# RobotLocomotion/pytorch-dense-correspondence

Measured on NVIDIA H100. Metric: image-pairs/s (640x480, D=3) fwd+loss+bwd, higher is better.
Workload: dtype f32 (bf16x3 split on the wgmma tensor cores, fp32 accumulate)

## Files before the change

### pytorch-dense-correspondence_b200/csrc/bn.cu

```cuda
#include "conv.cuh"

namespace ddn {

constexpr int BN_THREADS = 256;

__device__ __forceinline__ void store_split4(__nv_bfloat16* hi, __nv_bfloat16* lo, int64_t i4, float4 v) {
  __nv_bfloat16 h0 = __float2bfloat16_rn(v.x), h1 = __float2bfloat16_rn(v.y), h2 = __float2bfloat16_rn(v.z), h3 = __float2bfloat16_rn(v.w);
  __nv_bfloat162 a = __halves2bfloat162(h0, h1), b = __halves2bfloat162(h2, h3);
  uint2 ho; ho.x = *reinterpret_cast<uint32_t*>(&a); ho.y = *reinterpret_cast<uint32_t*>(&b);
  reinterpret_cast<uint2*>(hi)[i4] = ho;
  if (lo) {
    __nv_bfloat162 c = __halves2bfloat162(__float2bfloat16_rn(v.x - __bfloat162float(h0)), __float2bfloat16_rn(v.y - __bfloat162float(h1)));
    __nv_bfloat162 d = __halves2bfloat162(__float2bfloat16_rn(v.z - __bfloat162float(h2)), __float2bfloat16_rn(v.w - __bfloat162float(h3)));
    uint2 l2; l2.x = *reinterpret_cast<uint32_t*>(&c); l2.y = *reinterpret_cast<uint32_t*>(&d);
    reinterpret_cast<uint2*>(lo)[i4] = l2;
  }
}
__device__ __forceinline__ float4 bf16x4_to_float4(uint2 h) {
  return make_float4(__uint_as_float(h.x << 16), __uint_as_float(h.x & 0xffff0000u), __uint_as_float(h.y << 16),
                     __uint_as_float(h.y & 0xffff0000u));
}
__device__ __forceinline__ void mask_from_bf16x4(uint2 h, float4& g) {
  if ((h.x & 0x8000u) || !(h.x & 0x7fffu)) g.x = 0.f;
  if ((h.x & 0x80000000u) || !(h.x & 0x7fff0000u)) g.y = 0.f;
// ... 252 lines not shown
    if (a.g_out) reinterpret_cast<float4*>(a.g_out)[i] = g;
    float4 d;
    d.x = k1.x * (g.x - mb.x - (v.x - mu.x) * is.x * mg.x);
    d.y = k1.y * (g.y - mb.y - (v.y - mu.y) * is.y * mg.y);
    d.z = k1.z * (g.z - mb.z - (v.z - mu.z) * is.z * mg.z);
    d.w = k1.w * (g.w - mb.w - (v.w - mu.w) * is.w * mg.w);
    if (a.dx) reinterpret_cast<float4*>(a.dx)[i] = d;
    if (a.dx_hi) store_split4(a.dx_hi, a.dx_lo, i, d);
  }
}

__global__ void __launch_bounds__(256)
stem_bn_relu_pool_kernel(const float* __restrict__ x, const float* __restrict__ mean, const float* __restrict__ invstd,
                         const float* __restrict__ gamma, const float* __restrict__ beta,
                         float* __restrict__ y, uint8_t* __restrict__ argmax, __nv_bfloat16* __restrict__ y_hi,
                         __nv_bfloat16* __restrict__ y_lo, int N, int Hc, int Wc, int C, int Hp, int Wp, int imgs_per_group) {
  pdl_prologue();
  const int q = C >> 2;
  const int64_t total = (int64_t)N * Hp * Wp * q;
  for (int64_t i = (int64_t)blockIdx.x * blockDim.x + threadIdx.x; i < total; i += (int64_t)gridDim.x * blockDim.x) {
    int c = (int)(i % q) << 2; int64_t t = i / q;
    int wp = (int)(t % Wp); t /= Wp;
    int hp = (int)(t % Hp); int n = (int)(t / Hp);
    const int so = (n / imgs_per_group) * C + c;
    float4 mu = *reinterpret_cast<const float4*>(mean + so), is = *reinterpret_cast<const float4*>(invstd + so);
    float4 ga = *reinterpret_cast<const float4*>(gamma + c), be = *reinterpret_cast<const float4*>(beta + c);
    float4 sc = make_float4(ga.x * is.x, ga.y * is.y, ga.z * is.z, ga.w * is.w);
    float4 best = make_float4(-INFINITY, -INFINITY, -INFINITY, -INFINITY);
    uchar4 arg = make_uchar4(0, 0, 0, 0);
#pragma unroll
    for (int r = 0; r < 3; ++r) {
      int h = 2 * hp - 1 + r;
      if (h < 0 || h >= Hc) continue;
#pragma unroll
      for (int s = 0; s < 3; ++s) {
        int w = 2 * wp - 1 + s;
        if (w < 0 || w >= Wc) continue;
        float4 v = __ldg(reinterpret_cast<const float4*>(x + (((int64_t)n * Hc + h) * Wc + w) * C + c));
        v.x = fmaxf(fmaf(v.x - mu.x, sc.x, be.x), 0.f); v.y = fmaxf(fmaf(v.y - mu.y, sc.y, be.y), 0.f);
        v.z = fmaxf(fmaf(v.z - mu.z, sc.z, be.z), 0.f); v.w = fmaxf(fmaf(v.w - mu.w, sc.w, be.w), 0.f);
        unsigned char k = (unsigned char)(r * 3 + s);
        if (v.x > best.x) { best.x = v.x; arg.x = k; }
        if (v.y > best.y) { best.y = v.y; arg.y = k; }
        if (v.z > best.z) { best.z = v.z; arg.z = k; }
        if (v.w > best.w) { best.w = v.w; arg.w = k; }
      }
    }
    if (y) reinterpret_cast<float4*>(y)[i] = best;
    reinterpret_cast<uchar4*>(argmax)[i] = arg;
    if (y_hi) store_split4(y_hi, y_lo, i, best);
  }
}

__global__ void __launch_bounds__(256)
stem_pool_relu_bwd_kernel(const float* __restrict__ dyp, const uint8_t* __restrict__ argmax, const float* __restrict__ x,
                          const float* __restrict__ mean, const float* __restrict__ invstd,
                          const float* __restrict__ gamma, const float* __restrict__ beta, float* __restrict__ g,
                          int N, int Hc, int Wc, int C, int Hp, int Wp, int imgs_per_group) {
  pdl_prologue();
  const int q = C >> 2;
  const int64_t total = (int64_t)N * Hc * Wc * q;
  for (int64_t i = (int64_t)blockIdx.x * blockDim.x + threadIdx.x; i < total; i += (int64_t)gridDim.x * blockDim.x) {
    int c = (int)(i % q) << 2; int64_t t = i / q;
    int w = (int)(t % Wc); t /= Wc;
    int h = (int)(t % Hc); int n = (int)(t / Hc);
    float4 acc = make_float4(0, 0, 0, 0);
    int hp0 = h >> 1, hp1 = (h + 1) >> 1, wp0 = w >> 1, wp1 = (w + 1) >> 1;
#pragma unroll
    for (int a = 0; a < 2; ++a) {
      int hp = a ? hp1 : hp0;
      if ((a && hp1 == hp0) || hp >= Hp) continue;
      int r = h - (2 * hp - 1);
#pragma unroll
      for (int b = 0; b < 2; ++b) {
        int wp = b ? wp1 : wp0;
        if ((b && wp1 == wp0) || wp >= Wp) continue;
        int s = w - (2 * wp - 1);
        unsigned char k = (unsigned char)(r * 3 + s);
        int64_t pi = (((int64_t)n * Hp + hp) * Wp + wp) * q + (c >> 2);
        uchar4 am = reinterpret_cast<const uchar4*>(argmax)[pi];
        float4 d = __ldg(reinterpret_cast<const float4*>(dyp) + pi);
        if (am.x == k) acc.x += d.x;
        if (am.y == k) acc.y += d.y;
        if (am.z == k) acc.z += d.z;
        if (am.w == k) acc.w += d.w;
      }
    }
    const int so = (n / imgs_per_group) * C + c;
    float4 mu = *reinterpret_cast<const float4*>(mean + so), is = *reinterpret_cast<const float4*>(invstd + so);
    float4 ga = *reinterpret_cast<const float4*>(gamma + c), be = *reinterpret_cast<const float4*>(beta + c);
    float4 v = __ldg(reinterpret_cast<const float4*>(x) + i);
    if (!(fmaf(v.x - mu.x, ga.x * is.x, be.x) > 0.f)) acc.x = 0.f;
    if (!(fmaf(v.y - mu.y, ga.y * is.y, be.y) > 0.f)) acc.y = 0.f;
    if (!(fmaf(v.z - mu.z, ga.z * is.z, be.z) > 0.f)) acc.z = 0.f;
    if (!(fmaf(v.w - mu.w, ga.w * is.w, be.w) > 0.f)) acc.w = 0.f;
    reinterpret_cast<float4*>(g)[i] = acc;
  }
}

bool bn_c_supported(int C) {
  return C >= 4 && C % 4 == 0 && (C <= BN_COLSUM_MAX_C ? BN_THREADS % (C / 4) == 0 : (C % BN_COLSUM_MAX_C == 0 && C <= 4096));
}

static int check_c(int C, int G, int64_t M) {
  DDN_CHECK_ARG(bn_c_supported(C), "BatchNorm kernels need C in {4..1024} with 256 %% (C/4) == 0, or a multiple of 1024 up to 4096 (got %d)", C);
  DDN_CHECK_ARG(G >= 1 && G <= BN_MAX_GROUPS && M % G == 0, "BatchNorm groups: need 1 <= G <= %d dividing the row count", BN_MAX_GROUPS);
  return 0;
}
template <typename K>
static int resident_blocks(K kernel, size_t smem) {
  int per_sm = 0;
  if (cudaOccupancyMaxActiveBlocksPerMultiprocessor(&per_sm, kernel, BN_THREADS, smem) != cudaSuccess || per_sm < 1) per_sm = 4;
  return per_sm * num_sms();
}
template <typename K>
static int ew_blocks(K kernel, size_t smem, int64_t total) {
  return (int)std::min<int64_t>(ceil_div(total, BN_THREADS), (int64_t)resident_blocks(kernel, smem));
}

int launch_bn_stats(const float* x, int64_t M, int C, int G, BnAccum acc, float* mean, float* invstd,
                    float* running_mean, float* running_var, float momentum, float eps, cudaStream_t st) {
  DDN_TRY(check_c(C, G, M));
  const int64_t Mg = M / G;
  const int resident = resident_blocks(bn_colsum_kernel<0>, 0);
  const int Cs = bn_slice_c(C), slices = C / Cs;
  BnColsumArgs a = {x, nullptr, nullptr, nullptr, nullptr, nullptr, nullptr, nullptr, Mg, C, bn_colsum_rows_per_block(Mg, C, G * slices, resident), 0, Cs};
  BnFwdFinal ff = {acc, mean, invstd, running_mean, running_var, Mg, G, C, momentum, eps};
  BnBwdFinal fb = {};
  dim3 grid((unsigned)bn_colsum_blocks(Mg, C, G * slices, resident), (unsigned)G, (unsigned)slices);
  DDN_LAUNCH(bn_colsum_kernel<0>, grid, BN_THREADS, 0, st, a, ff, fb);
  return 0;
}

int launch_bn_eval_stats(const float* rm, const float* rv, int C, int G, float eps, float* mean, float* invstd, cudaStream_t st) {
  DDN_LAUNCH(bn_eval_stats_kernel, (int)ceil_div(C, 128), 128, 0, st, rm, rv, C, G, eps, mean, invstd);
  return 0;
}

int launch_bn_eval_stats_all(const float* buffers, float* stats_base, const BnEvalSeg* segs, int n_segs, int G, float eps, cudaStream_t st) {
  DDN_CHECK_ARG(n_segs >= 1, "no BatchNorm segments");
  for (int i0 = 0; i0 < n_segs; i0 += BN_EVAL_MAX_SEGS) {
    BnEvalSegs s; s.n = std::min(BN_EVAL_MAX_SEGS, n_segs - i0);
    for (int i = 0; i < s.n; ++i) s.s[i] = segs[i0 + i];
    dim3 grid(2, (unsigned)s.n);
    DDN_LAUNCH(bn_eval_stats_all_kernel, grid, 256, 0, st, buffers, stats_base, s, G, eps);
  }
  return 0;
}

int launch_bn_fold(const float* rm, const float* rv, const float* gamma, const float* beta, int C, float eps,
                   float* scale, float* shift, cudaStream_t st) {
  DDN_LAUNCH(bn_fold_kernel, (int)ceil_div(C, 128), 128, 0, st, rm, rv, gamma, beta, C, eps, scale, shift);
  return 0;
}

template <typename K>
static int allow_smem(K kernel, size_t smem) {
  if (smem > 48 * 1024) DDN_CUDA(cudaFuncSetAttribute(kernel, cudaFuncAttributeMaxDynamicSharedMemorySize, (int)smem));
  return 0;
}

int launch_bn_apply(const BnApplyArgs& a, cudaStream_t st) {
  DDN_TRY(check_c(a.C, a.G, a.M));
  const size_t smem = (size_t)a.G * ((a.r && a.rmean) ? 6 : 3) * a.C * sizeof(float);
  DDN_TRY(allow_smem(bn_apply_kernel, smem));
  DDN_LAUNCH(bn_apply_kernel, ew_blocks(bn_apply_kernel, smem, a.M * (a.C / 4)), BN_THREADS, smem, st, a);
  return 0;
}

int launch_bn_backward(const BnBwdArgs& a, cudaStream_t st) {
  DDN_TRY(check_c(a.C, a.G, a.M));
  const int64_t Mg = a.M / a.G;
  const int resident = resident_blocks(bn_colsum_kernel<1>, 0);
  const int Cs = bn_slice_c(a.C), slices = a.C / Cs;
  BnColsumArgs ca = {a.x, a.dy, a.y, a.y_hi, a.mean, a.invstd, a.gamma, a.beta, Mg, a.C, bn_colsum_rows_per_block(Mg, a.C, a.G * slices, resident),
                     a.relu, Cs};
  DDN_CHECK_ARG(!(a.relu && !a.y && !a.y_hi) || a.beta, "recomputing the ReLU mask needs beta");
  BnFwdFinal ff = {};
  BnBwdFinal fb = {a.acc, a.sums, a.dgamma, a.dbeta, a.G, a.C};
  dim3 grid((unsigned)bn_colsum_blocks(Mg, a.C, a.G * slices, resident), (unsigned)a.G, (unsigned)slices);
  if (!a.sums_ready) DDN_LAUNCH(bn_colsum_kernel<1>, grid, BN_THREADS, 0, st, ca, ff, fb);
  const size_t smem = (size_t)a.G * 7 * a.C * sizeof(float);
  DDN_TRY(allow_smem(bn_bwd_apply_kernel, smem));
  DDN_LAUNCH(bn_bwd_apply_kernel, ew_blocks(bn_bwd_apply_kernel, smem, a.M * (a.C / 4)), BN_THREADS, smem, st, a);
  return 0;
}

int launch_stem_bn_relu_pool(const float* x, const float* mean, const float* invstd, const float* gamma, const float* beta,
                             float* y, uint8_t* argmax, __nv_bfloat16* y_hi, __nv_bfloat16* y_lo,
                             int N, int Hc, int Wc, int C, int G, cudaStream_t st) {
  int Hp = (Hc - 1) / 2 + 1, Wp = (Wc - 1) / 2 + 1;
  int64_t total = (int64_t)N * Hp * Wp * (C / 4);
  DDN_LAUNCH(stem_bn_relu_pool_kernel, ew_blocks(stem_bn_relu_pool_kernel, 0, total), 256, 0, st, x, mean, invstd, gamma, beta, y, argmax, y_hi, y_lo, N, Hc, Wc, C,
             Hp, Wp, N / G);
  return 0;
}

int launch_stem_pool_relu_backward(const float* dy_pool, const uint8_t* argmax, const float* x, const float* mean,
                                   const float* invstd, const float* gamma, const float* beta, float* g,
                                   int N, int Hc, int Wc, int C, int G, cudaStream_t st) {
  int Hp = (Hc - 1) / 2 + 1, Wp = (Wc - 1) / 2 + 1;
  int64_t total = (int64_t)N * Hc * Wc * (C / 4);
  DDN_LAUNCH(stem_pool_relu_bwd_kernel, ew_blocks(stem_pool_relu_bwd_kernel, 0, total), 256, 0, st, dy_pool, argmax, x, mean, invstd, gamma, beta, g,
             N, Hc, Wc, C, Hp, Wp, N / G);
  return 0;
}

}
```

### pytorch-dense-correspondence_b200/csrc/conv.cuh

```cuda
#pragma once
#include "common.cuh"
#include "bn_stats.cuh"

namespace ddn {

struct ConvGeom {
  int N, Hin, Win, Cin;
  int Hout, Wout, Cout;
  int KH, KW;
  int stride;
  int ups;
  int pad, dil;
  int cin_log2;
};

int conv_geom_init(ConvGeom* g, int N, int Hin, int Win, int Cin, int Hout, int Wout, int Cout,
                   int KH, int KW, int stride, int ups, int pad, int dil);
int launch_pack_weights(const float* w, float* wp, int Cout, int Cin, int CinP, int KH, int KW, int dgrad, cudaStream_t st);
int launch_unpack_wgrad(const float* dwp, float* dw, int Cout, int Cin, int CinP, int KH, int KW, cudaStream_t st);
int launch_conv_gather_f32(const float* in, const float* wp, const float* addend, float* out, const ConvGeom& g, cudaStream_t st);
int launch_conv_wgrad_f32(const float* in, const float* dy, float* dwp, const ConvGeom& g, cudaStream_t st);

bool bn_c_supported(int C);
size_t bn_accum_bytes(int C);
BnAccum bn_accum_at(void* base, int C);
int launch_bn_stats(const float* x, int64_t M, int C, int G, BnAccum acc, float* mean, float* invstd,
                    float* running_mean, float* running_var, float momentum, float eps, cudaStream_t st);
struct BnEvalSeg { int64_t rm_off, rv_off, stat_off; int C; };
int launch_bn_eval_stats_all(const float* buffers, float* stats_base, const BnEvalSeg* segs, int n_segs, int G, float eps, cudaStream_t st);
int launch_bn_eval_stats(const float* running_mean, const float* running_var, int C, int G, float eps,
                         float* mean, float* invstd, cudaStream_t st);
int launch_bn_fold(const float* running_mean, const float* running_var, const float* gamma, const float* beta, int C, float eps,
                   float* scale, float* shift, cudaStream_t st);
struct BnApplyArgs {
  const float* x; const float* mean; const float* invstd; const float* gamma; const float* beta;
  const float* r; const __nv_bfloat16* r_hi; const __nv_bfloat16* r_lo;
  const float* rmean; const float* rinvstd; const float* rgamma; const float* rbeta;
  float* y; __nv_bfloat16* hi; __nv_bfloat16* lo;
  int64_t M; int C; int relu; int G;
};
int launch_bn_apply(const BnApplyArgs& a, cudaStream_t st);
struct BnBwdArgs {
  const float* dy; const float* x; const float* mean; const float* invstd; const float* gamma; const float* beta;
  const float* y; const __nv_bfloat16* y_hi;
  float* dx; __nv_bfloat16* dx_hi; __nv_bfloat16* dx_lo; float* g_out;
  float* dgamma; float* dbeta;
  BnAccum acc; float* sums;
  int64_t M; int C; int relu; int training; int G;
  int sums_ready;
};
int launch_bn_backward(const BnBwdArgs& a, cudaStream_t st);

int launch_stem_bn_relu_pool(const float* x, const float* mean, const float* invstd, const float* gamma, const float* beta,
                             float* y, uint8_t* argmax, __nv_bfloat16* y_hi, __nv_bfloat16* y_lo,
                             int N, int Hc, int Wc, int C, int G, cudaStream_t st);
int launch_stem_pool_relu_backward(const float* dy_pool, const uint8_t* argmax, const float* x, const float* mean,
                                   const float* invstd, const float* gamma, const float* beta, float* g,
                                   int N, int Hc, int Wc, int C, int G, cudaStream_t st);

int launch_nchw_to_nhwc4(const float* x, float* y, int N, int H, int W, cudaStream_t st);
int launch_fc_forward(const float* feat, const __nv_bfloat16* feat_hi, const __nv_bfloat16* feat_lo, const float* w, const float* bias,
                      float* low, float* low_nhwc, int64_t Mimg, int N, int C, int D, cudaStream_t st);
int launch_add_lowres_nhwc(const float* dlow_nhwc, float* dlow, int64_t Mimg, int N, int D, int accumulate, cudaStream_t st);
size_t fc_part_floats(int C, int D);
int launch_fc_backward(const float* dlow, const float* feat, const __nv_bfloat16* feat_hi, const __nv_bfloat16* feat_lo, const float* w,
                       float* dfeat, float* dw, float* dbias, float* part, int64_t Mimg, int N, int C, int D, cudaStream_t st);
int launch_upsample_fwd(const float* x, float* y, int NC, int h, int w, int H, int W, cudaStream_t st);
int launch_upsample_bwd(const float* dy, float* dx, int NC, int h, int w, int H, int W, cudaStream_t st);
int launch_upsample_unit_fwd(const float* x, float* y, int N, int D, int h, int w, int H, int W, cudaStream_t st);
int launch_upsample_unit_bwd(const float* x, const float* dy, float* dx, float* g, int N, int D, int h, int w, int H, int W, cudaStream_t st);
int launch_fill_zero(void* p, size_t bytes, cudaStream_t st);

}
```

### pytorch-dense-correspondence_b200/csrc/conv_tc.cu

```cuda
#include <cuda.h>
#include <algorithm>
#include <cstring>
#include <functional>
#include <mutex>
#include <unordered_map>

#include "conv.cuh"
#include "conv_tc.cuh"

namespace ddn {

constexpr int TC_BLOCK_K = 64;
constexpr int TC_CONSUMERS = 256;
constexpr int TC_THREADS = TC_CONSUMERS + 32;
constexpr int TC_PRODUCER_WARP = TC_CONSUMERS / 32;
constexpr int TC_WIDE_THREADS = TC_CONSUMERS + 128;
constexpr int TC_A_BYTES = 128 * TC_BLOCK_K * 2;

__device__ __forceinline__ uint32_t smem_u32(const void* p) { return (uint32_t)__cvta_generic_to_shared(p); }

__device__ __forceinline__ void mbar_init(uint32_t bar, uint32_t count) {
  asm volatile("mbarrier.init.shared::cta.b64 [%0], %1;" ::"r"(bar), "r"(count));
}
__device__ __forceinline__ void mbar_expect_tx(uint32_t bar, uint32_t bytes) {
// ... 169 lines not shown
  const float* addend;
  int imgs_per_group;
  BnFwdFinal fin;
  TcBwdStats bst;
  const float* ep_scale; const float* ep_shift; int ep_relu;
  __nv_bfloat16* out_hi; __nv_bfloat16* out_lo;
};

__device__ __forceinline__ void conv_epilogue_rows(const TcEpilogueParams& p, const float4 (&v)[EPI_ROWS], size_t off, size_t rs, int n_ok, int ch,
                                                   int C, int grp, float4& s1, float4& s2) {
  float4 adv[EPI_ROWS];
#pragma unroll
  for (int i = 0; i < EPI_ROWS; ++i)
    adv[i] = (p.addend && i < n_ok) ? __ldg(reinterpret_cast<const float4*>(p.addend + off + i * rs)) : make_float4(0.f, 0.f, 0.f, 0.f);
  if (p.ep_scale) {
    const float4 sc = __ldg(reinterpret_cast<const float4*>(p.ep_scale + ch));
    const float4 sh = __ldg(reinterpret_cast<const float4*>(p.ep_shift + ch));
#pragma unroll
    for (int i = 0; i < EPI_ROWS; ++i) {
      float4 f = make_float4(fmaf(v[i].x, sc.x, sh.x) + adv[i].x, fmaf(v[i].y, sc.y, sh.y) + adv[i].y,
                             fmaf(v[i].z, sc.z, sh.z) + adv[i].z, fmaf(v[i].w, sc.w, sh.w) + adv[i].w);
      if (p.ep_relu) { f.x = fmaxf(f.x, 0.f); f.y = fmaxf(f.y, 0.f); f.z = fmaxf(f.z, 0.f); f.w = fmaxf(f.w, 0.f); }
      if (i < n_ok) {
        if (p.out) *reinterpret_cast<float4*>(p.out + off + i * rs) = f;
        if (p.out_hi) {
          const __nv_bfloat16 h0 = __float2bfloat16_rn(f.x), h1 = __float2bfloat16_rn(f.y), h2 = __float2bfloat16_rn(f.z), h3 = __float2bfloat16_rn(f.w);
          *reinterpret_cast<uint2*>(p.out_hi + off + i * rs) = make_uint2(pack_bf16x2(h0, h1), pack_bf16x2(h2, h3));
          if (p.out_lo)
            *reinterpret_cast<uint2*>(p.out_lo + off + i * rs) =
                make_uint2(pack_bf16x2(__float2bfloat16_rn(f.x - __bfloat162float(h0)), __float2bfloat16_rn(f.y - __bfloat162float(h1))),
                           pack_bf16x2(__float2bfloat16_rn(f.z - __bfloat162float(h2)), __float2bfloat16_rn(f.w - __bfloat162float(h3))));
        }
      }
    }
  } else if (p.bst.fin.a.acc) {
    float4 rw[EPI_ROWS];
    uint2 yh[EPI_ROWS];
#pragma unroll
    for (int i = 0; i < EPI_ROWS; ++i) {
      rw[i] = i < n_ok ? __ldg(reinterpret_cast<const float4*>(p.bst.raw + off + i * rs)) : make_float4(0.f, 0.f, 0.f, 0.f);
      if (p.bst.y_hi) yh[i] = i < n_ok ? __ldg(reinterpret_cast<const uint2*>(p.bst.y_hi + off + i * rs)) : make_uint2(0u, 0u);
    }
    const float4 mu = __ldg(reinterpret_cast<const float4*>(p.bst.mean + (size_t)grp * C + ch));
    const float4 is = __ldg(reinterpret_cast<const float4*>(p.bst.invstd + (size_t)grp * C + ch));
    float4 scl = make_float4(0.f, 0.f, 0.f, 0.f), be = scl;
    if (!p.bst.y_hi && p.bst.relu) {
      const float4 gm = __ldg(reinterpret_cast<const float4*>(p.bst.gamma + ch));
      be = __ldg(reinterpret_cast<const float4*>(p.bst.beta + ch));
      scl = make_float4(gm.x * is.x, gm.y * is.y, gm.z * is.z, gm.w * is.w);
    }
#pragma unroll
    for (int i = 0; i < EPI_ROWS; ++i) {
      float4 g = make_float4(v[i].x + adv[i].x, v[i].y + adv[i].y, v[i].z + adv[i].z, v[i].w + adv[i].w);
      if (i < n_ok) *reinterpret_cast<float4*>(p.out + off + i * rs) = g;
      else g = make_float4(0.f, 0.f, 0.f, 0.f);
      if (p.bst.y_hi) {
        const uint2 hh = yh[i];
        if ((hh.x & 0x8000u) || !(hh.x & 0x7fffu)) g.x = 0.f;
        if ((hh.x & 0x80000000u) || !(hh.x & 0x7fff0000u)) g.y = 0.f;
        if ((hh.y & 0x8000u) || !(hh.y & 0x7fffu)) g.z = 0.f;
        if ((hh.y & 0x80000000u) || !(hh.y & 0x7fff0000u)) g.w = 0.f;
      } else if (p.bst.relu) {
        if (!(fmaf(rw[i].x - mu.x, scl.x, be.x) > 0.f)) g.x = 0.f;
        if (!(fmaf(rw[i].y - mu.y, scl.y, be.y) > 0.f)) g.y = 0.f;
        if (!(fmaf(rw[i].z - mu.z, scl.z, be.z) > 0.f)) g.z = 0.f;
        if (!(fmaf(rw[i].w - mu.w, scl.w, be.w) > 0.f)) g.w = 0.f;
      }
      s1.x += g.x; s1.y += g.y; s1.z += g.z; s1.w += g.w;
      s2.x = fmaf(g.x, (rw[i].x - mu.x) * is.x, s2.x); s2.y = fmaf(g.y, (rw[i].y - mu.y) * is.y, s2.y);
      s2.z = fmaf(g.z, (rw[i].z - mu.z) * is.z, s2.z); s2.w = fmaf(g.w, (rw[i].w - mu.w) * is.w, s2.w);
    }
  } else {
#pragma unroll
    for (int i = 0; i < EPI_ROWS; ++i) {
      const float4 raw = i < n_ok ? v[i] : make_float4(0.f, 0.f, 0.f, 0.f);
      if (i < n_ok)
        *reinterpret_cast<float4*>(p.out + off + i * rs) = make_float4(raw.x + adv[i].x, raw.y + adv[i].y, raw.z + adv[i].z, raw.w + adv[i].w);
      s1.x += raw.x; s1.y += raw.y; s1.z += raw.z; s1.w += raw.w;
      s2.x = fmaf(raw.x, raw.x, s2.x); s2.y = fmaf(raw.y, raw.y, s2.y); s2.z = fmaf(raw.z, raw.z, s2.z); s2.w = fmaf(raw.w, raw.w, s2.w);
    }
  }
}

__device__ __forceinline__ void colsum_lane_groups(float4& s1, float4& s2) {
#pragma unroll
  for (int off = 8; off < 32; off <<= 1) {
    s1.x += __shfl_xor_sync(0xffffffffu, s1.x, off); s1.y += __shfl_xor_sync(0xffffffffu, s1.y, off);
    s1.z += __shfl_xor_sync(0xffffffffu, s1.z, off); s1.w += __shfl_xor_sync(0xffffffffu, s1.w, off);
    s2.x += __shfl_xor_sync(0xffffffffu, s2.x, off); s2.y += __shfl_xor_sync(0xffffffffu, s2.y, off);
    s2.z += __shfl_xor_sync(0xffffffffu, s2.z, off); s2.w += __shfl_xor_sync(0xffffffffu, s2.w, off);
  }
}

__device__ __forceinline__ void named_barrier(int id, int threads) { asm volatile("bar.sync %0, %1;" ::"r"(id), "r"(threads) : "memory"); }

__device__ __forceinline__ void conv_epilogue_finalize(const TcEpilogueParams& p, int C, int* s_last, int bar) {
  if (p.fin.a.acc) {
    if (bn_last_cta(p.fin.a.ticket, gridDim.x, threadIdx.x == 0, s_last, [bar] { named_barrier(bar, TC_CONSUMERS); }))
      for (int c = threadIdx.x; c < C; c += TC_CONSUMERS) bn_fwd_finalize_channel(p.fin, c);
  } else if (p.bst.fin.a.acc) {
    if (bn_last_cta(p.bst.fin.a.ticket, gridDim.x, threadIdx.x == 0, s_last, [bar] { named_barrier(bar, TC_CONSUMERS); }))
      for (int c = threadIdx.x; c < C; c += TC_CONSUMERS) bn_bwd_finalize_channel(p.bst.fin, c);
  }
}

struct TcConvParams {
  TcEpilogueParams epi;
  int N, H, W, Cin, Cout;
  int taps_w;
  int dil;
  int stride;
  int tiles_h, tiles_w;
  int n_sub;
  int n_co;
  int full_items, tail_split, total_items;
};

constexpr int TC_SUB_H = 4, TC_SUB_W = 16;
constexpr int TC_SUB_BYTES = 64 * 128;

// ... 1258 lines not shown
```

### pytorch-dense-correspondence_b200/csrc/conv_tc.cuh

```cuda
#pragma once
#include "common.cuh"
#include "bn_stats.cuh"

namespace ddn {

struct TcPlanes { const __nv_bfloat16* hi; const __nv_bfloat16* lo; };

struct TcFoldedEpilogue { const float* scale; const float* shift; int relu; __nv_bfloat16* out_hi; __nv_bfloat16* out_lo; };

struct TcBwdStats {
  const float* raw; const __nv_bfloat16* y_hi;
  const float* mean; const float* invstd;
  const float* gamma; const float* beta;
  int relu;
  BnBwdFinal fin;
};

bool tc_conv_supported(int Cin, int Cout, int k, int stride, int pad, int dil, int H, int W);
size_t tc_weight_ws_bytes();
size_t tc_max_weight_elems();
size_t tc_workspace_bytes(size_t max_act_elems);
int tc_split(const float* x, __nv_bfloat16* hi, __nv_bfloat16* lo, int64_t n, int precision, cudaStream_t st);

int tc_conv_planes(TcPlanes in, const float* w_oihw, const TcPlanes* w_packed, float* out, const float* addend, const BnFwdFinal* stats,
                   int N, int H, int W, int Cin, int Cout, int k, int stride, int dil, int dgrad, int precision,
                   void* wws, size_t wws_bytes, cudaStream_t st, const TcFoldedEpilogue* ep = nullptr, const TcBwdStats* bst = nullptr);
int tc_dgrad_strided(const float* dy_f32, TcPlanes up, const float* w_oihw, const TcPlanes* w_packed, float* dx, const float* addend,
                     int N, int H, int W, int Cin, int Cout, int k, int precision, void* wws, size_t wws_bytes, cudaStream_t st,
                     const TcBwdStats* bst = nullptr);
int tc_wgrad_planes(TcPlanes x, TcPlanes dy, float* dw, int N, int H, int W, int Cin, int Cout, int k, int stride, int dil,
                    int precision, double* dwp, cudaStream_t st);
struct TcUnpackEntry { int64_t src_off, dst_off; int Cout, Cin, taps, kind; };
constexpr int TC_UNPACK_MAX = 40;
struct TcUnpackTable { TcUnpackEntry e[TC_UNPACK_MAX]; int n; };
int tc_unpack_wgrads(const TcUnpackEntry* entries, int n, const double* dwp_base, float* grads_base, cudaStream_t st);
struct TcPackEntry { int64_t w_off, dst_off; int Cout, Cin, k, dgrad, kind; };
constexpr int TC_PACK_MAX = 80;
struct TcPackTable { TcPackEntry e[TC_PACK_MAX]; int n; };
int tc_pack_all(const float* params, int64_t n_params, char* cache, const TcPackEntry* entries, int n, unsigned long long* fp_new,
                unsigned long long* fp_old, int force, int precision, cudaStream_t st);
int tc_stem_patches(const float* x_nchw, __nv_bfloat16* hi, __nv_bfloat16* lo, int N, int H, int W, int precision, cudaStream_t st);
int tc_stem_pack_weights(const float* w_conv1, __nv_bfloat16* hi, __nv_bfloat16* lo, int precision, cudaStream_t st);
int tc_stem_forward(TcPlanes patches, const float* w_conv1, const TcPlanes* w_packed, float* raw, const BnFwdFinal* stats, int N, int H1,
                    int W1, int precision, void* wws, size_t wws_bytes, cudaStream_t st);
int tc_stem_wgrad(TcPlanes patches, TcPlanes dy, int N, int H1, int W1, int precision, double* dwp, cudaStream_t st);

int stage_planes(void* ws, size_t ws_bytes, size_t x_el, size_t dy_el, size_t up_el, void** wws, TcPlanes* x, TcPlanes* dy, TcPlanes* up);
int tc_conv_forward(const float* x_nhwc, const float* w_oihw, float* y_nhwc, int N, int H, int W, int Cin, int Cout,
                    int k, int stride, int pad, int dil, int precision, void* ws, size_t ws_bytes, cudaStream_t st);
int tc_conv_backward(const float* x_nhwc, const float* w_oihw, const float* dy_nhwc, float* dx_nhwc, const float* dx_addend,
                     float* dw_oihw, int N, int H, int W, int Cin, int Cout, int k, int stride, int pad, int dil, int precision,
                     void* ws, size_t ws_bytes, double* dwp_scratch, cudaStream_t st);

}
```

### pytorch-dense-correspondence_b200/csrc/engine.cu

```cuda
#include <algorithm>
#include <cstring>
#include <deque>
#include <mutex>
#include <string>
#include <vector>

#include "conv.cuh"
#include "conv_tc.cuh"

namespace ddn {

std::atomic<long long> g_launches{0};
static thread_local char g_err[512] = "";

void set_error(const char* fmt, ...) {
  va_list ap;
  va_start(ap, fmt);
  vsnprintf(g_err, sizeof(g_err), fmt, ap);
  va_end(ap);
}

static std::atomic<int> g_reserved_sms{-1};
static std::atomic<int> g_window_reserved{0};
static int overlap_window_sms() {
// ... 487 lines not shown
}

static int simt_wgrad(const float* in, const float* dy, float* dwp, float* dw, int N, int Hin, int Win, int cin, int cin_eff, int Hout,
                      int Wout, int cout, int k, int stride, int pad, int dil, cudaStream_t st) {
  ConvGeom g;
  DDN_TRY(conv_geom_init(&g, N, Hin, Win, cin_eff, Hout, Wout, cout, k, k, stride, 1, pad, dil));
  DDN_TRY(launch_fill_zero(dwp, sizeof(float) * (size_t)k * k * cin_eff * cout, st));
  {
    ProfScope ps(PROF_CONV_WGRAD_SIMT, 2.0 * N * Hout * Wout * (double)cout * k * k * cin, st);
    DDN_TRY(launch_conv_wgrad_f32(in, dy, dwp, g, st));
  }
  return launch_unpack_wgrad(dwp, dw, cout, cin, cin_eff, k, k, st);
}

static int conv_backward(const Ctx& c, const ConvSpec& cs, const float* in, const PlaneBufs& in_p, const float* dy, float* dx,
                         const float* addend, int N, int Hin, int Win, int Hout, int Wout, int cin_eff, const TcBwdStats* bst = nullptr) {
  const Plan& p = *c.p;
  const float* w = c.params + cs.w_off;
  float* dw = c.grads + cs.w_off;
  const double fl = 2.0 * N * Hout * Wout * (double)cs.cout * cs.k * cs.k * cs.cin;
  if (p.tc) {
    DDN_TRY(tc_wgrad_planes(c.planes(in_p), c.planes(p.grad_p), nullptr, N, Hin, Win, cs.cin, cs.cout, cs.k, cs.stride, cs.dil,
                            p.precision, c.d(p.dwp_all) + cs.w_off, c.st));
    if (dx) {
      TcPlanes wpk_s; const TcPlanes* wpk = cached_pack(c, cs, 1, &wpk_s);
      if (cs.stride == 2)
        DDN_TRY(tc_dgrad_strided(dy, c.planes(p.grad_p), w, wpk, dx, addend, N, Hin, Win, cs.cin, cs.cout, cs.k, p.precision,
                                 c.ws + p.wws, tc_weight_ws_bytes(), c.st, bst));
      else
        DDN_TRY(tc_conv_planes(c.planes(p.grad_p), w, wpk, dx, addend, nullptr, N, Hin, Win, cs.cin, cs.cout, cs.k, 1, cs.dil, 1,
                               p.precision, c.ws + p.wws, tc_weight_ws_bytes(), c.st, nullptr, bst));
    }
    return 0;
  }
  DDN_CHECK_ARG(bst == nullptr, "backward statistics can only ride on a tensor-core data gradient");
  DDN_TRY(simt_wgrad(in, dy, c.f(p.dwp), dw, N, Hin, Win, cs.cin, cin_eff, Hout, Wout, cs.cout, cs.k, cs.stride, cs.pad, cs.dil, c.st));
  if (dx) {
    ConvGeom gd;
    DDN_TRY(conv_geom_init(&gd, N, Hout, Wout, cs.cout, Hin, Win, cs.cin, cs.k, cs.k, 1, cs.stride, cs.dil * (cs.k - 1) - cs.pad, cs.dil));
    DDN_TRY(launch_pack_weights(w, c.f(p.wpack2), cs.cout, cs.cin, cs.cin, cs.k, cs.k, 1, c.st));
    ProfScope ps(PROF_CONV_DGRAD_SIMT, fl, c.st);
    DDN_TRY(launch_conv_gather_f32(dy, c.f(p.wpack2), addend, dx, gd, c.st));
  }
  return 0;
}

static int bn_backward_for(const Ctx& c, const BnSpec& bs, const ConvBufs& cb, const float* dy, const float* y_f32,
                           const __nv_bfloat16* y_hi, int relu, float* g_out, const ConvSpec& cs, float* dx_f32, int64_t M,
                           int fused_slot = 0) {
  BnBwdArgs a;
  memset(&a, 0, sizeof(a));
  a.dy = dy; a.x = c.f(cb.raw); a.mean = c.mean(cb.stats); a.invstd = c.invstd(cb.stats, bs.C);
  a.gamma = c.params + bs.g_off; a.beta = c.params + bs.b_off;
  a.y = y_f32; a.y_hi = y_hi; a.g_out = g_out;
  a.dgamma = c.grads + bs.g_off; a.dbeta = c.grads + bs.b_off;
  a.acc = c.accum(); a.sums = c.sums(fused_slot);
  a.sums_ready = fused_slot > 0;
  a.M = M; a.C = bs.C; a.relu = relu; a.training = c.training() ? 1 : 0; a.G = c.G;
  if (c.p->tc) {
    a.dx = cs.stride == 2 ? dx_f32 : nullptr;
    a.dx_hi = c.h(c.p->grad_p.hi);
    a.dx_lo = c.p->precision == DDN_PRECISION_BF16X3 ? c.h(c.p->grad_p.lo) : nullptr;
  } else {
    a.dx = dx_f32;
  }
  return launch_bn_backward(a, c.st);
}

static bool bwd_stats_for(const Ctx& c, const BnSpec& bs, const ConvBufs& cb, const __nv_bfloat16* y_hi, int slot, TcBwdStats* out) {
  if (!c.p->tc) return false;
  memset(out, 0, sizeof(*out));
  out->raw = c.f(cb.raw); out->y_hi = y_hi; out->mean = c.mean(cb.stats); out->invstd = c.invstd(cb.stats, bs.C);
  out->gamma = c.params + bs.g_off; out->beta = c.params + bs.b_off; out->relu = 1;
  out->fin.a = c.accum(); out->fin.sums = c.sums(slot);
  out->fin.dgamma = c.grads + bs.g_off; out->fin.dbeta = c.grads + bs.b_off; out->fin.G = c.G; out->fin.C = bs.C;
  return true;
}

struct StemBwdArgs {
  const float* dy_pool; const uint8_t* argmax;
  const float* raw; const float* mean; const float* invstd;
  const float* gamma; const float* beta; float* dgamma; float* dbeta;
  float* g;
  float* dx;
  BnAccum acc; float* sums;
  TcPlanes patches; __nv_bfloat16* dx_hi; __nv_bfloat16* dx_lo; double* dwp;
  const float* x4; float* dwp_f32; float* dw;
  int N, H, W, H1, W1, G, training, precision;
};

static int stem_backward(const StemBwdArgs& a, cudaStream_t st) {
  DDN_TRY(launch_stem_pool_relu_backward(a.dy_pool, a.argmax, a.raw, a.mean, a.invstd, a.gamma, a.beta, a.g, a.N, a.H1, a.W1, 64, a.G, st));
  const bool tc = a.precision != DDN_PRECISION_FP32_SIMT;
  BnBwdArgs ks;
  memset(&ks, 0, sizeof(ks));
  ks.dy = a.g; ks.x = a.raw; ks.mean = a.mean; ks.invstd = a.invstd; ks.gamma = a.gamma; ks.beta = a.beta;
  ks.dgamma = a.dgamma; ks.dbeta = a.dbeta; ks.acc = a.acc; ks.sums = a.sums;
  ks.M = (int64_t)a.N * a.H1 * a.W1; ks.C = 64; ks.relu = 0; ks.training = a.training; ks.G = a.G;
  ks.dx = a.dx;
  if (tc) { ks.dx_hi = a.dx_hi; ks.dx_lo = a.precision == DDN_PRECISION_BF16X3 ? a.dx_lo : nullptr; }
  DDN_TRY(launch_bn_backward(ks, st));
  if (tc) return tc_stem_wgrad(a.patches, TcPlanes{a.dx_hi, a.dx_lo}, a.N, a.H1, a.W1, a.precision, a.dwp, st);
  return simt_wgrad(a.x4, a.dx, a.dwp_f32, a.dw, a.N, a.H, a.W, 3, 4, a.H1, a.W1, 64, 7, 2, 3, 1, st);
}

static TcUnpackEntry stem_unpack_entry(int64_t src_off, int64_t dst_off) {
  TcUnpackEntry e; e.src_off = src_off; e.dst_off = dst_off; e.Cout = 64; e.Cin = 3; e.taps = 49; e.kind = 1;
  return e;
}

struct Bucket { int64_t begin, end; };

static int net_backward(const Ctx& c, const float* dy, const float* dlow_nhwc, ddn_grad_bucket_fn on_bucket, void* user) {
  const NetSpec& s = *c.s; const Plan& p = *c.p;
  const int B = p.B, h8 = p.H / 8, w8 = p.W / 8;
  const bool want_lo = p.precision == DDN_PRECISION_BF16X3;
  float* S[4] = {c.f(p.scratch[0]), c.f(p.scratch[1]), c.f(p.scratch[2]), c.f(p.scratch[3])};
  DDN_CUDA(cudaMemsetAsync(c.ws + p.acc, 0, bn_accum_bytes(s.max_c), c.st));
  if (p.tc) DDN_CUDA(cudaMemsetAsync(c.d(p.dwp_all), 0, sizeof(double) * (size_t)(s.n_params + 64 * 192), c.st));
  const BlockBufs& last = p.blk.back();
  if (dy && (p.flags & DDN_NET_UNIT_DESCRIPTORS))
    DDN_TRY(launch_upsample_unit_bwd(c.f(p.low), dy, c.f(p.dlow), c.f(p.unit_dy), B, p.D, h8, w8, p.H, p.W, c.st));
  else if (dy)
    DDN_TRY(launch_upsample_bwd(dy, c.f(p.dlow), B * p.D, h8, w8, p.H, p.W, c.st));
  if (dlow_nhwc) DDN_TRY(launch_add_lowres_nhwc(dlow_nhwc, c.f(p.dlow), (int64_t)h8 * w8, B, p.D, dy ? 1 : 0, c.st));
  int cur = 0;
  DDN_TRY(launch_fc_backward(c.f(p.dlow), p.tc ? nullptr : c.f(last.out), p.tc ? c.h(last.out_p.hi) : nullptr,
                             (p.tc && want_lo) ? c.h(last.out_p.lo) : nullptr, c.params + s.fc_w, S[cur], c.grads + s.fc_w,
                             c.grads + s.fc_b, c.f(p.fc_part), (int64_t)h8 * w8, B, s.fc_cin, p.D, c.st));
  std::vector<TcUnpackEntry> pending;
  auto defer = [&](const ConvSpec& cs) {
    if (!p.tc) return;
    TcUnpackEntry e; e.src_off = cs.w_off; e.dst_off = cs.w_off; e.Cout = cs.cout; e.Cin = cs.cin; e.taps = cs.k * cs.k; e.kind = 0;
    pending.push_back(e);
  };
  int64_t bucket_end = s.n_params;
  int bucket_id = 0;
  struct WindowGuard { ~WindowGuard() { g_window_reserved.store(0, std::memory_order_relaxed); } } window_guard;
  auto close_bucket = [&](int64_t begin) -> int {
    if (!pending.empty()) DDN_TRY(tc_unpack_wgrads(pending.data(), (int)pending.size(), c.d(p.dwp_all), c.grads, c.st));
    pending.clear();
    if (on_bucket) {
      on_bucket(user, bucket_id, begin, bucket_end - begin);
      g_window_reserved.store(overlap_window_sms(), std::memory_order_relaxed);
    }
    ++bucket_id; bucket_end = begin;
    return 0;
  };
  bool out_fused = false;
  for (int i = (int)s.blocks.size() - 1; i >= 0; --i) {
    const BlockSpec& b = s.blocks[i]; const BlockBufs& bb = p.blk[i];
    const int last = b.n - 1;
    const float* xin = p.tc ? nullptr : (i == 0 ? c.f(p.pool_out) : c.f(p.blk[i - 1].out));
    const PlaneBufs xin_p = i == 0 ? p.pool_p : p.blk[i - 1].out_p;
    auto rows = [&](const ConvBufs& cb) { return (int64_t)B * cb.Hout * cb.Wout; };
    int t1 = (cur + 1) & 3, t2 = (cur + 2) & 3, t3 = (cur + 3) & 3;
    DDN_TRY(bn_backward_for(c, b.b[last], bb.c[last], S[cur], p.tc ? nullptr : c.f(bb.out), p.tc ? c.h(bb.out_p.hi) : nullptr, 1, S[t2],
                            b.c[last], S[t1], rows(bb.c[last]), out_fused ? 2 : 0));
    TcBwdStats st_in, st_next;
    bool in_fused = false;
    for (int j = last; j >= 1; --j) {
      in_fused = bwd_stats_for(c, b.b[j - 1], bb.c[j - 1], nullptr, 1, &st_in);
      DDN_TRY(conv_backward(c, b.c[j], p.tc ? nullptr : c.f(bb.act[j - 1]), bb.act_p[j - 1], S[t1], S[t3], nullptr, B, bb.c[j].Hin,
                            bb.c[j].Win, bb.c[j].Hout, bb.c[j].Wout, b.c[j].cin, in_fused ? &st_in : nullptr));
      defer(b.c[j]);
      if (j > 1)
        DDN_TRY(bn_backward_for(c, b.b[j - 1], bb.c[j - 1], S[t3], p.tc ? nullptr : c.f(bb.act[j - 1]), nullptr, 1, nullptr, b.c[j - 1],
                                S[t1], rows(bb.c[j - 1]), in_fused ? 1 : 0));
    }
    out_fused = i > 0 && bwd_stats_for(c, s.blocks[i - 1].b[last], p.blk[i - 1].c[last], c.h(p.blk[i - 1].out_p.hi), 2, &st_next);
    if (!b.has_ds) {
      DDN_TRY(bn_backward_for(c, b.b[0], bb.c[0], S[t3], p.tc ? nullptr : c.f(bb.act[0]), nullptr, 1, nullptr, b.c[0], S[t1],
                              rows(bb.c[0]), in_fused ? 1 : 0));
      DDN_TRY(conv_backward(c, b.c[0], xin, xin_p, S[t1], S[t3], S[t2], B, bb.c[0].Hin, bb.c[0].Win, bb.c[0].Hout, bb.c[0].Wout, b.c[0].cin,
                            out_fused ? &st_next : nullptr));
      defer(b.c[0]);
      cur = t3;
    } else {
      DDN_TRY(bn_backward_for(c, b.bd, bb.ds, S[t2], nullptr, nullptr, 0, nullptr, b.ds, S[t1], rows(bb.ds)));
      DDN_TRY(conv_backward(c, b.ds, xin, xin_p, S[t1], S[cur], nullptr, B, bb.ds.Hin, bb.ds.Win, bb.ds.Hout, bb.ds.Wout, b.ds.cin));
      defer(b.ds);
      DDN_TRY(bn_backward_for(c, b.b[0], bb.c[0], S[t3], p.tc ? nullptr : c.f(bb.act[0]), nullptr, 1, nullptr, b.c[0], S[t1],
                              rows(bb.c[0]), in_fused ? 1 : 0));
      DDN_TRY(conv_backward(c, b.c[0], xin, xin_p, S[t1], S[t2], S[cur], B, bb.c[0].Hin, bb.c[0].Win, bb.c[0].Hout, bb.c[0].Wout, b.c[0].cin,
                            out_fused ? &st_next : nullptr));
      defer(b.c[0]);
      cur = t2;
      if (i > 0) DDN_TRY(close_bucket(b.c[0].w_off));
    }
  }
  StemBwdArgs sa;
  memset(&sa, 0, sizeof(sa));
  sa.dy_pool = S[cur]; sa.argmax = reinterpret_cast<const uint8_t*>(c.ws + p.argmax);
  sa.raw = c.f(p.stem_raw); sa.mean = c.mean(p.stem_stats); sa.invstd = c.invstd(p.stem_stats, 64);
  sa.gamma = c.params + s.stem_bn.g_off; sa.beta = c.params + s.stem_bn.b_off;
  sa.dgamma = c.grads + s.stem_bn.g_off; sa.dbeta = c.grads + s.stem_bn.b_off;
  sa.g = S[(cur + 1) & 3]; sa.acc = c.accum(); sa.sums = c.f(p.sums);
  sa.N = B; sa.H = p.H; sa.W = p.W; sa.H1 = p.H1; sa.W1 = p.W1; sa.G = c.G; sa.training = c.training() ? 1 : 0; sa.precision = p.precision;
  if (p.tc) {
    sa.patches = c.planes(p.patch_p); sa.dx_hi = c.h(p.grad_p.hi); sa.dx_lo = c.h(p.grad_p.lo); sa.dwp = c.d(p.dwp_all) + s.n_params;
  } else {
    sa.dx = S[(cur + 2) & 3]; sa.x4 = c.f(p.x4); sa.dwp_f32 = c.f(p.dwp); sa.dw = c.grads + s.stem.w_off;
  }
  DDN_TRY(stem_backward(sa, c.st));
  if (p.tc) pending.push_back(stem_unpack_entry(s.n_params, s.stem.w_off));
  return close_bucket(0);
}

}

using namespace ddn;

extern "C" int ddn_abi_version(void) { return DDN_ABI_VERSION; }
extern "C" int ddn_set_reserved_sms(int n) {
  DDN_CHECK_ARG(n >= 0 && n <= 64, "reserved SM count must be in [0, 64]");
  g_reserved_sms.store(n);
  return 0;
}
extern "C" const char* ddn_last_error(void) { return g_err; }
extern "C" int64_t ddn_kernel_launch_count(void) { return g_launches.load(); }

extern "C" int ddn_profile_enable(int on) { g_prof_on.store(on ? 1 : 0); return 0; }
extern "C" int ddn_profile_reset(void) {
  std::lock_guard<std::mutex> lk(g_prof_mu);
  g_prof_used = 0;
  return 0;
}
extern "C" int ddn_profile_read(ddn_profile_entry* out, int cap) {
  std::lock_guard<std::mutex> lk(g_prof_mu);
  double ms[PROF_NUM_CLASSES] = {0}, work[PROF_NUM_CLASSES] = {0};
  int64_t n[PROF_NUM_CLASSES] = {0};
  for (size_t i = 0; i < g_prof_used; ++i) {
// ... 448 lines not shown
```

Before: 140.1.

## Fuse stem BN backward reductions into pool backward and store masked residual grads

The stem max-pool/ReLU backward kernel now accumulates the BatchNorm dgamma/dbeta column sums per group and finalizes them in the last CTA, so the following BN backward skips its separate column-sum pass. In the residual block backward, the conv epilogue that already fuses stats now stores the ReLU-masked gradient directly into the current buffer. The BN backward call for fused slots then skips re-masking and the extra copy into another scratch buffer. This removes a reduction kernel and some memory traffic, at the cost of a 2D grid with per-group blocks, double-precision atomics, and more complex buffer aliasing.

```diff
diff --git a/pytorch-dense-correspondence_b200/csrc/bn.cu b/pytorch-dense-correspondence_b200/csrc/bn.cu
--- a/pytorch-dense-correspondence_b200/csrc/bn.cu
+++ b/pytorch-dense-correspondence_b200/csrc/bn.cu
@@ -328,15 +328,19 @@
   }
 }
 
-__global__ void __launch_bounds__(256)
+__global__ void __launch_bounds__(BN_THREADS)
 stem_pool_relu_bwd_kernel(const float* __restrict__ dyp, const uint8_t* __restrict__ argmax, const float* __restrict__ x,
                           const float* __restrict__ mean, const float* __restrict__ invstd,
                           const float* __restrict__ gamma, const float* __restrict__ beta, float* __restrict__ g,
-                          int N, int Hc, int Wc, int C, int Hp, int Wp, int imgs_per_group) {
+                          int N, int Hc, int Wc, int C, int Hp, int Wp, int imgs_per_group, BnBwdFinal fb) {
   pdl_prologue();
   const int q = C >> 2;
-  const int64_t total = (int64_t)N * Hc * Wc * q;
-  for (int64_t i = (int64_t)blockIdx.x * blockDim.x + threadIdx.x; i < total; i += (int64_t)gridDim.x * blockDim.x) {
+  const int grp = blockIdx.y;
+  const int64_t per_group = (int64_t)imgs_per_group * Hc * Wc * q;
+  const int64_t end = (int64_t)(grp + 1) * per_group;
+  const int cq = threadIdx.x % q;
+  float4 s0 = make_float4(0.f, 0.f, 0.f, 0.f), s1 = s0;
+  for (int64_t i = grp * per_group + (int64_t)blockIdx.x * blockDim.x + threadIdx.x; i < end; i += (int64_t)gridDim.x * blockDim.x) {
     int c = (int)(i % q) << 2; int64_t t = i / q;
     int w = (int)(t % Wc); t /= Wc;
     int h = (int)(t % Hc); int n = (int)(t / Hc);
@@ -371,7 +375,27 @@
     if (!(fmaf(v.z - mu.z, ga.z * is.z, be.z) > 0.f)) acc.z = 0.f;
     if (!(fmaf(v.w - mu.w, ga.w * is.w, be.w) > 0.f)) acc.w = 0.f;
     reinterpret_cast<float4*>(g)[i] = acc;
-  }
+    s0.x += acc.x; s0.y += acc.y; s0.z += acc.z; s0.w += acc.w;
+    s1.x = fmaf(acc.x, (v.x - mu.x) * is.x, s1.x); s1.y = fmaf(acc.y, (v.y - mu.y) * is.y, s1.y);
+    s1.z = fmaf(acc.z, (v.z - mu.z) * is.z, s1.z); s1.w = fmaf(acc.w, (v.w - mu.w) * is.w, s1.w);
+  }
+  __shared__ float4 sh0[BN_THREADS], sh1[BN_THREADS];
+  __shared__ int s_last;
+  sh0[threadIdx.x] = s0; sh1[threadIdx.x] = s1;
+  __syncthreads();
+  if (threadIdx.x < q) {
+    for (int k = 1; k < BN_THREADS / q; ++k) {
+      const float4 u = sh0[k * q + threadIdx.x], w = sh1[k * q + threadIdx.x];
+      s0.x += u.x; s0.y += u.y; s0.z += u.z; s0.w += u.w;
+      s1.x += w.x; s1.y += w.y; s1.z += w.z; s1.w += w.w;
+    }
+    double* p0 = fb.a.acc + (size_t)(grp * 2) * C + (cq << 2);
+    double* p1 = p0 + C;
+    red_add_f64(p0, (double)s0.x); red_add_f64(p0 + 1, (double)s0.y); red_add_f64(p0 + 2, (double)s0.z); red_add_f64(p0 + 3, (double)s0.w);
+    red_add_f64(p1, (double)s1.x); red_add_f64(p1 + 1, (double)s1.y); red_add_f64(p1 + 2, (double)s1.z); red_add_f64(p1 + 3, (double)s1.w);
+  }
+  if (bn_last_cta(fb.a.ticket, gridDim.x * gridDim.y, threadIdx.x == 0, &s_last, [] { __syncthreads(); }))
+    for (int c = threadIdx.x; c < C; c += BN_THREADS) bn_bwd_finalize_channel(fb, c);
 }
 
 bool bn_c_supported(int C) {
@@ -473,13 +497,17 @@
 }
 
 int launch_stem_pool_relu_backward(const float* dy_pool, const uint8_t* argmax, const float* x, const float* mean,
-                                   const float* invstd, const float* gamma, const float* beta, float* g,
+                                   const float* invstd, const float* gamma, const float* beta, float* g, const BnBwdFinal& fin,
                                    int N, int Hc, int Wc, int C, int G, cudaStream_t st) {
+  DDN_CHECK_ARG(C >= 4 && C % 4 == 0 && BN_THREADS % (C / 4) == 0, "stem pool backward: C = %d does not tile a block", C);
+  DDN_CHECK_ARG(G >= 1 && G <= BN_MAX_GROUPS && N % G == 0 && fin.G == G && fin.C == C && fin.a.acc, "stem pool backward: bad BatchNorm request");
   int Hp = (Hc - 1) / 2 + 1, Wp = (Wc - 1) / 2 + 1;
-  int64_t total = (int64_t)N * Hc * Wc * (C / 4);
-  DDN_LAUNCH(stem_pool_relu_bwd_kernel, ew_blocks(stem_pool_relu_bwd_kernel, 0, total), 256, 0, st, dy_pool, argmax, x, mean, invstd, gamma, beta, g,
-             N, Hc, Wc, C, Hp, Wp, N / G);
-  return 0;
-}
-
-}
+  const int64_t per_group = (int64_t)(N / G) * Hc * Wc * (C / 4);
+  const int blocks = (int)std::max<int64_t>(1, std::min<int64_t>(ceil_div(per_group, BN_THREADS),
+                                                                 resident_blocks(stem_pool_relu_bwd_kernel, 0) / G));
+  DDN_LAUNCH(stem_pool_relu_bwd_kernel, dim3((unsigned)blocks, (unsigned)G), BN_THREADS, 0, st, dy_pool, argmax, x, mean, invstd, gamma, beta, g,
+             N, Hc, Wc, C, Hp, Wp, N / G, fin);
+  return 0;
+}
+
+}
diff --git a/pytorch-dense-correspondence_b200/csrc/conv.cuh b/pytorch-dense-correspondence_b200/csrc/conv.cuh
--- a/pytorch-dense-correspondence_b200/csrc/conv.cuh
+++ b/pytorch-dense-correspondence_b200/csrc/conv.cuh
@@ -55,7 +55,7 @@
                              float* y, uint8_t* argmax, __nv_bfloat16* y_hi, __nv_bfloat16* y_lo,
                              int N, int Hc, int Wc, int C, int G, cudaStream_t st);
 int launch_stem_pool_relu_backward(const float* dy_pool, const uint8_t* argmax, const float* x, const float* mean,
-                                   const float* invstd, const float* gamma, const float* beta, float* g,
+                                   const float* invstd, const float* gamma, const float* beta, float* g, const BnBwdFinal& fin,
                                    int N, int Hc, int Wc, int C, int G, cudaStream_t st);
 
 int launch_nchw_to_nhwc4(const float* x, float* y, int N, int H, int W, cudaStream_t st);
diff --git a/pytorch-dense-correspondence_b200/csrc/conv_tc.cu b/pytorch-dense-correspondence_b200/csrc/conv_tc.cu
--- a/pytorch-dense-correspondence_b200/csrc/conv_tc.cu
+++ b/pytorch-dense-correspondence_b200/csrc/conv_tc.cu
@@ -245,8 +245,8 @@
 #pragma unroll
     for (int i = 0; i < EPI_ROWS; ++i) {
       float4 g = make_float4(v[i].x + adv[i].x, v[i].y + adv[i].y, v[i].z + adv[i].z, v[i].w + adv[i].w);
-      if (i < n_ok) *reinterpret_cast<float4*>(p.out + off + i * rs) = g;
-      else g = make_float4(0.f, 0.f, 0.f, 0.f);
+      if (i >= n_ok) g = make_float4(0.f, 0.f, 0.f, 0.f);
+      else if (!p.bst.store_masked) *reinterpret_cast<float4*>(p.out + off + i * rs) = g;
       if (p.bst.y_hi) {
         const uint2 hh = yh[i];
         if ((hh.x & 0x8000u) || !(hh.x & 0x7fffu)) g.x = 0.f;
@@ -259,6 +259,7 @@
         if (!(fmaf(rw[i].z - mu.z, scl.z, be.z) > 0.f)) g.z = 0.f;
         if (!(fmaf(rw[i].w - mu.w, scl.w, be.w) > 0.f)) g.w = 0.f;
       }
+      if (p.bst.store_masked && i < n_ok) *reinterpret_cast<float4*>(p.out + off + i * rs) = g;
       s1.x += g.x; s1.y += g.y; s1.z += g.z; s1.w += g.w;
       s2.x = fmaf(g.x, (rw[i].x - mu.x) * is.x, s2.x); s2.y = fmaf(g.y, (rw[i].y - mu.y) * is.y, s2.y);
       s2.z = fmaf(g.z, (rw[i].z - mu.z) * is.z, s2.z); s2.w = fmaf(g.w, (rw[i].w - mu.w) * is.w, s2.w);
diff --git a/pytorch-dense-correspondence_b200/csrc/conv_tc.cuh b/pytorch-dense-correspondence_b200/csrc/conv_tc.cuh
--- a/pytorch-dense-correspondence_b200/csrc/conv_tc.cuh
+++ b/pytorch-dense-correspondence_b200/csrc/conv_tc.cuh
@@ -13,6 +13,7 @@
   const float* mean; const float* invstd;
   const float* gamma; const float* beta;
   int relu;
+  int store_masked;
   BnBwdFinal fin;
 };
 
diff --git a/pytorch-dense-correspondence_b200/csrc/engine.cu b/pytorch-dense-correspondence_b200/csrc/engine.cu
--- a/pytorch-dense-correspondence_b200/csrc/engine.cu
+++ b/pytorch-dense-correspondence_b200/csrc/engine.cu
@@ -563,7 +563,8 @@
   memset(&a, 0, sizeof(a));
   a.dy = dy; a.x = c.f(cb.raw); a.mean = c.mean(cb.stats); a.invstd = c.invstd(cb.stats, bs.C);
   a.gamma = c.params + bs.g_off; a.beta = c.params + bs.b_off;
-  a.y = y_f32; a.y_hi = y_hi; a.g_out = g_out;
+  if (fused_slot > 0) relu = 0;
+  else { a.y = y_f32; a.y_hi = y_hi; a.g_out = g_out; }
   a.dgamma = c.grads + bs.g_off; a.dbeta = c.grads + bs.b_off;
   a.acc = c.accum(); a.sums = c.sums(fused_slot);
   a.sums_ready = fused_slot > 0;
@@ -582,7 +583,7 @@
   if (!c.p->tc) return false;
   memset(out, 0, sizeof(*out));
   out->raw = c.f(cb.raw); out->y_hi = y_hi; out->mean = c.mean(cb.stats); out->invstd = c.invstd(cb.stats, bs.C);
-  out->gamma = c.params + bs.g_off; out->beta = c.params + bs.b_off; out->relu = 1;
+  out->gamma = c.params + bs.g_off; out->beta = c.params + bs.b_off; out->relu = 1; out->store_masked = 1;
   out->fin.a = c.accum(); out->fin.sums = c.sums(slot);
   out->fin.dgamma = c.grads + bs.g_off; out->fin.dbeta = c.grads + bs.b_off; out->fin.G = c.G; out->fin.C = bs.C;
   return true;
@@ -601,12 +602,13 @@
 };
 
 static int stem_backward(const StemBwdArgs& a, cudaStream_t st) {
-  DDN_TRY(launch_stem_pool_relu_backward(a.dy_pool, a.argmax, a.raw, a.mean, a.invstd, a.gamma, a.beta, a.g, a.N, a.H1, a.W1, 64, a.G, st));
+  const BnBwdFinal fin = {a.acc, a.sums, a.dgamma, a.dbeta, a.G, 64};
+  DDN_TRY(launch_stem_pool_relu_backward(a.dy_pool, a.argmax, a.raw, a.mean, a.invstd, a.gamma, a.beta, a.g, fin, a.N, a.H1, a.W1, 64, a.G, st));
   const bool tc = a.precision != DDN_PRECISION_FP32_SIMT;
   BnBwdArgs ks;
   memset(&ks, 0, sizeof(ks));
   ks.dy = a.g; ks.x = a.raw; ks.mean = a.mean; ks.invstd = a.invstd; ks.gamma = a.gamma; ks.beta = a.beta;
-  ks.dgamma = a.dgamma; ks.dbeta = a.dbeta; ks.acc = a.acc; ks.sums = a.sums;
+  ks.dgamma = a.dgamma; ks.dbeta = a.dbeta; ks.acc = a.acc; ks.sums = a.sums; ks.sums_ready = 1;
   ks.M = (int64_t)a.N * a.H1 * a.W1; ks.C = 64; ks.relu = 0; ks.training = a.training; ks.G = a.G;
   ks.dx = a.dx;
   if (tc) { ks.dx_hi = a.dx_hi; ks.dx_lo = a.precision == DDN_PRECISION_BF16X3 ? a.dx_lo : nullptr; }
@@ -666,7 +668,8 @@
     const PlaneBufs xin_p = i == 0 ? p.pool_p : p.blk[i - 1].out_p;
     auto rows = [&](const ConvBufs& cb) { return (int64_t)B * cb.Hout * cb.Wout; };
     int t1 = (cur + 1) & 3, t2 = (cur + 2) & 3, t3 = (cur + 3) & 3;
-    DDN_TRY(bn_backward_for(c, b.b[last], bb.c[last], S[cur], p.tc ? nullptr : c.f(bb.out), p.tc ? c.h(bb.out_p.hi) : nullptr, 1, S[t2],
+    float* const g = out_fused ? S[cur] : S[t2];
+    DDN_TRY(bn_backward_for(c, b.b[last], bb.c[last], S[cur], p.tc ? nullptr : c.f(bb.out), p.tc ? c.h(bb.out_p.hi) : nullptr, 1, g,
                             b.c[last], S[t1], rows(bb.c[last]), out_fused ? 2 : 0));
     TcBwdStats st_in, st_next;
     bool in_fused = false;
@@ -683,12 +686,12 @@
     if (!b.has_ds) {
       DDN_TRY(bn_backward_for(c, b.b[0], bb.c[0], S[t3], p.tc ? nullptr : c.f(bb.act[0]), nullptr, 1, nullptr, b.c[0], S[t1],
                               rows(bb.c[0]), in_fused ? 1 : 0));
-      DDN_TRY(conv_backward(c, b.c[0], xin, xin_p, S[t1], S[t3], S[t2], B, bb.c[0].Hin, bb.c[0].Win, bb.c[0].Hout, bb.c[0].Wout, b.c[0].cin,
+      DDN_TRY(conv_backward(c, b.c[0], xin, xin_p, S[t1], S[t3], g, B, bb.c[0].Hin, bb.c[0].Win, bb.c[0].Hout, bb.c[0].Wout, b.c[0].cin,
                             out_fused ? &st_next : nullptr));
       defer(b.c[0]);
       cur = t3;
     } else {
-      DDN_TRY(bn_backward_for(c, b.bd, bb.ds, S[t2], nullptr, nullptr, 0, nullptr, b.ds, S[t1], rows(bb.ds)));
+      DDN_TRY(bn_backward_for(c, b.bd, bb.ds, g, nullptr, nullptr, 0, nullptr, b.ds, S[t1], rows(bb.ds)));
       DDN_TRY(conv_backward(c, b.ds, xin, xin_p, S[t1], S[cur], nullptr, B, bb.ds.Hin, bb.ds.Win, bb.ds.Hout, bb.ds.Wout, b.ds.cin));
       defer(b.ds);
       DDN_TRY(bn_backward_for(c, b.b[0], bb.c[0], S[t3], p.tc ? nullptr : c.f(bb.act[0]), nullptr, 1, nullptr, b.c[0], S[t1],
```

Result: faster. 142.4 (median of 6 runs) (+1.7%).
